# mokemokechicken/reversi-alpha-zero

Hardware: AMD Instinct MI355X
Metric: MCTS simulations/sec (self-play, NN included) (higher is better)
Workload: dtype f64 tree statistics + f32 net (f16x3 split-operand MFMA trunk)

## Files before the change

### reversi-alpha-zero_amd/csrc/raz_net_f16x3.hip

```cpp
#include <hip/hip_runtime.h>
#include <math.h>
#include <stdlib.h>
#include <string.h>
#include <vector>
#include "raz_bitboard.h"
#include "raz_detmath.h"
#include "raz_internal.h"
#include "raz_net_heads.h"
#include "raz_net_layout.h"

namespace {

typedef _Float16 h8 __attribute__((ext_vector_type(8)));
typedef _Float16 h4 __attribute__((ext_vector_type(4)));
typedef float f32x4 __attribute__((ext_vector_type(4)));
typedef float f32x16 __attribute__((ext_vector_type(16)));

constexpr int OCT = 128;
constexpr int NWAVE = 8;
constexpr int W_STAGE = 3 * 2 * 2 * OCT * 16;
constexpr int ACT_POS = 4 * 64 * 16;
constexpr int Z_OFF = NWAVE * (ACT_POS + 128);
constexpr int Z_BYTES = 2048;
constexpr int ACT_IMG = Z_OFF + Z_BYTES;
constexpr int LDS_W = 0;
constexpr int LDS_ACT = 2 * W_STAGE;
constexpr int LDS_BYTES = LDS_ACT + 2 * ACT_IMG;
constexpr int act_pos_off(int p) { return p * (ACT_POS + 128); }

#ifdef RAZ_F16X3_STAMPS
#define RAZ_STAMP_PARAM , unsigned long long* __restrict__ stamps
#define RAZ_STAMP_ARG , (unsigned long long*)nullptr
#define RAZ_STAMP_BEGIN                                                                                           \
    unsigned long long st_t[8];                                                                                   \
    st_t[0] = __builtin_amdgcn_s_memtime();                                                                       \
    st_t[7] = __builtin_amdgcn_s_memrealtime();                                                                   \
    st_t[6] = (unsigned long long)__builtin_amdgcn_s_getreg((4 << 0) | (0 << 6) | (31 << 11)) | ((unsigned long long)__builtin_amdgcn_s_getreg((20 << 0) | (0 << 6) | (31 << 11)) << 32); \
    st_t[5] = 0;                                                                                                  \
    st_t[1] = st_t[2] = st_t[3] = st_t[4] = 0;                                                                    \
    unsigned long long st_b = 0
#define RAZ_STAMP_BARRIER_IN st_b = __builtin_amdgcn_s_memtime()
#define RAZ_STAMP_BARRIER_OUT(st_)                                    \
    do {                                                              \
        const unsigned long long t_ = __builtin_amdgcn_s_memtime();   \
        st_t[5] += t_ - st_b;                                         \
        if ((st_) == 0) st_t[1] = t_;                                 \
    } while (0)
#define RAZ_STAMP_AT(i_) st_t[i_] = __builtin_amdgcn_s_memtime()
#define RAZ_STAMP_END                                                                                    \
    do {                                                                                                 \
        st_t[3] = __builtin_amdgcn_s_memtime();                                                          \
        __builtin_amdgcn_s_waitcnt(0x0070);                                                \
        st_t[4] = __builtin_amdgcn_s_memtime();                                                          \
        if (lane == 0 && stamps)                                                                         \
            for (int i_ = 0; i_ < 8; ++i_) stamps[((size_t)blockIdx.x * NWAVE + wv) * 8 + i_] = st_t[i_]; \
    } while (0)
#else
#define RAZ_STAMP_PARAM
#define RAZ_STAMP_ARG
#define RAZ_STAMP_BEGIN
#define RAZ_STAMP_BARRIER_IN
#define RAZ_STAMP_BARRIER_OUT(st_)
#define RAZ_STAMP_AT(i_)
#define RAZ_STAMP_END
#endif

__device__ __forceinline__ void halves_trade(float a, float b, int upper, float& first, float& second) {
#ifdef RAZ_WAVE_EMU
    const float got = __shfl_xor(upper ? a : b, 32);
    first = upper ? got : a;
    second = upper ? b : got;
#else
    (void)upper;
    const auto r = __builtin_amdgcn_permlane32_swap(__float_as_uint(a), __float_as_uint(b), false, false);
    first = __uint_as_float(r[0]);
    second = __uint_as_float(r[1]);
#endif
}

#define GLDS16(gptr, lptr)                                                                                      \
    __builtin_amdgcn_global_load_lds((const __attribute__((address_space(1))) void*)(gptr),                     \
                                     (__attribute__((address_space(3))) void*)(lptr), 16, 0, 0)

template <bool SPLIT, int TG, int J0, int J1>
__device__ __forceinline__ void conv_stage(const unsigned char* lds, uint32_t wbase, uint32_t abase, const uint32_t (&boff)[3],
                                           f32x16 (&acc)[2][4]) {
#pragma unroll
    for (int tt = 0; tt < 3; ++tt) {
        h8 bh[4], bl[4];
#pragma unroll
        for (int j = J0; j < J1; ++j) {
            const uint32_t at = abase + boff[tt] + (j + TG) * 128;
            bh[j] = *(const h8*)(lds + at);
            if constexpr (SPLIT) bl[j] = *(const h8*)(lds + at + 1024);
        }
#pragma unroll
        for (int m = 0; m < 2; ++m) {
            const h8 ah = *(const h8*)(lds + wbase + tt * 8192 + m * 512);
            if constexpr (SPLIT) {
                const h8 al = *(const h8*)(lds + wbase + tt * 8192 + m * 512 + 2048);
#pragma unroll
                for (int j = J0; j < J1; ++j) {
                    acc[m][j] = __builtin_amdgcn_mfma_f32_32x32x16_f16(al, bh[j], acc[m][j], 0, 0, 0);
                    acc[m][j] = __builtin_amdgcn_mfma_f32_32x32x16_f16(ah, bl[j], acc[m][j], 0, 0, 0);
                    acc[m][j] = __builtin_amdgcn_mfma_f32_32x32x16_f16(ah, bh[j], acc[m][j], 0, 0, 0);
                }
            } else {
#pragma unroll
                for (int j = J0; j < J1; ++j) acc[m][j] = __builtin_amdgcn_mfma_f32_32x32x16_f16(ah, bh[j], acc[m][j], 0, 0, 0);
            }
        }
    }
}

template <bool SPLIT>
__global__ __launch_bounds__(512, 2) void k_conv3x3_f16x3(const unsigned char* __restrict__ Wl, const float* __restrict__ bias,
                                                          const float* __restrict__ inv_scale_ptr, const unsigned char* in, unsigned char* out,
                                                          const unsigned char* skip, const uint8_t* __restrict__ active, int n, int F,
                                                          unsigned* __restrict__ flag, const uint32_t* __restrict__ n_ptr RAZ_STAMP_PARAM) {
    extern __shared__ __attribute__((aligned(16))) unsigned char lds[];
    const int tid = threadIdx.x, lane = tid & 63;
    const int wv = __builtin_amdgcn_readfirstlane(tid >> 6);
    RAZ_STAMP_BEGIN;
    if (n_ptr) n = (int)*n_ptr < n ? (int)*n_ptr : n;
    const int noct = F / OCT, nchunks = F / 16;
    const int b = blockIdx.x;
    const int ot = (b >> 3) % noct;
    const int pg = (b / (8 * noct)) * 8 + (b & 7);
    const int p0 = pg * NWAVE, pos = p0 + wv;
    if (p0 >= n) return;
    const size_t pos_bytes = (size_t)F * 256;
    const unsigned char* in_pos = in + (size_t)(pos < n ? pos : n - 1) * pos_bytes;
    if (tid < 2 * (Z_BYTES / 16)) {
        const int im = tid / (Z_BYTES / 16), k = tid % (Z_BYTES / 16);
        ((f32x4*)(lds + LDS_ACT + im * ACT_IMG + Z_OFF))[k] = (f32x4){0.f, 0.f, 0.f, 0.f};
    }
    const int half = wv >> 2, grp = (wv >> 1) & 1, oh = wv & 1;
    const int kg = lane >> 5, colpos = grp * 4 + ((lane & 31) >> 3), x = lane & 7;
    uint32_t boff[3];
#pragma unroll
    for (int t = 0; t < 3; ++t) {
        const int xx = x + t - 1;
        const int at = act_pos_off(colpos) + kg * 2048 + ((4 * half - 1) * 8 + xx) * 16;
        boff[t] = xx >= 0 && xx < 8 ? (uint32_t)at : (uint32_t)(Z_OFF + (at & 255));
    }
    const uint32_t aoff = (uint32_t)(kg * 4096 + oh * 1024 + (lane & 31) * 16);
    f32x16 acc[2][4];
#pragma unroll
    for (int m = 0; m < 2; ++m)
#pragma unroll
        for (int j = 0; j < 4; ++j)
#pragma unroll
            for (int r = 0; r < 16; ++r) acc[m][j][r] = 0.f;
    const unsigned char* wsrc = Wl + (size_t)ot * nchunks * 3 * W_STAGE + lane * 16;
    const unsigned char* asrc = in_pos + lane * 16;
    auto issue = [&](int c, int tg) {
        const int st = c * 3 + tg;
        const unsigned char* src = wsrc + (size_t)st * W_STAGE;
        unsigned char* dst = lds + LDS_W + (st & 1) * W_STAGE;
        if constexpr (SPLIT) {
#pragma unroll
            for (int i = 0; i < 3; ++i) GLDS16(src + (wv * 3 + i) * 1024, dst + (wv * 3 + i) * 1024);
        } else {
            const int p0w = (wv >> 1) * 4 + (wv & 1);
            GLDS16(src + p0w * 1024, dst + p0w * 1024);
            if (wv < 4) GLDS16(src + (p0w + 16) * 1024, dst + (p0w + 16) * 1024);
        }
        if (tg == 0) {
            const unsigned char* a = asrc + (size_t)c * ACT_POS;
            unsigned char* ad = lds + LDS_ACT + (c & 1) * ACT_IMG + act_pos_off(wv);
#pragma unroll
            for (int pl = 0; pl < 4; pl += SPLIT ? 1 : 2) GLDS16(a + pl * 1024, ad + pl * 1024);
        }
    };
    issue(0, 0);
    for (int c = 0; c < nchunks; ++c) {
        const uint32_t abase = (uint32_t)(LDS_ACT + (c & 1) * ACT_IMG);
#pragma unroll
        for (int tg = 0; tg < 3; ++tg) {
            const int st = c * 3 + tg;
            RAZ_STAMP_BARRIER_IN;
            __syncthreads();
            RAZ_STAMP_BARRIER_OUT(st);
            if (tg < 2) issue(c, tg + 1);
            else if (c + 1 < nchunks) issue(c + 1, 0);
            const uint32_t wbase = (uint32_t)(LDS_W + (st & 1) * W_STAGE) + aoff;
            if (tg == 0) {
                conv_stage<SPLIT, 0, 1, 4>(lds, wbase, abase, boff, acc);
                if (half != 0) conv_stage<SPLIT, 0, 0, 1>(lds, wbase, abase, boff, acc);
            } else if (tg == 1) {
                conv_stage<SPLIT, 1, 0, 4>(lds, wbase, abase, boff, acc);
            } else {
                conv_stage<SPLIT, 2, 0, 3>(lds, wbase, abase, boff, acc);
                if (half != 1) conv_stage<SPLIT, 2, 3, 4>(lds, wbase, abase, boff, acc);
            }
        }
    }
    RAZ_STAMP_AT(2);
    const int lpos = p0 + colpos;
    const bool live = lpos < n && (!active || active[lpos]);
    if (!__any(live)) return;
    const float inv_scale = *inv_scale_ptr;
    const size_t lane_off = (size_t)(live ? lpos : p0) * pos_bytes + (size_t)((4 * half + kg) * 8 + x) * 16;
    unsigned char* out_pos = out + lane_off;
    const unsigned char* skip_pos = skip ? skip + lane_off : nullptr;
    h8 skh[2][4], skl[2][4];
    auto load_skip = [&](int it) {
#pragma unroll
        for (int q = 0; q < 4; ++q) {
            const int oc8 = ot * OCT + oh * 64 + (it >> 1) * 32 + q * 8;
            const size_t unit = (size_t)(oc8 >> 4) * ACT_POS + (size_t)((oc8 >> 3) & 1) * 2048 + (size_t)(it & 1) * 256;
            skh[it & 1][q] = *(const h8*)(skip_pos + unit);
            if constexpr (SPLIT) skl[it & 1][q] = *(const h8*)(skip_pos + unit + 1024);
        }
    };
    if (skip_pos && live) load_skip(0);
    bool over = false;
#pragma unroll
    for (int it = 0; it < 4; ++it) {
        const int m = it >> 1, k = it & 1;
        if (skip_pos && live && it + 1 < 4) load_skip(it + 1);
#pragma unroll
        for (int q = 0; q < 4; ++q) {
            const int oc8 = ot * OCT + oh * 64 + m * 32 + q * 8;
            const size_t unit = (size_t)(oc8 >> 4) * ACT_POS + (size_t)((oc8 >> 3) & 1) * 2048 + (size_t)k * 256;
            float v[8];
#pragma unroll
            for (int j = 0; j < 4; ++j) halves_trade(acc[m][2 * k][q * 4 + j], acc[m][2 * k + 1][q * 4 + j], kg, v[j], v[4 + j]);
            if (!live) continue;
#pragma unroll
            for (int j = 0; j < 8; ++j) v[j] = v[j] * inv_scale + bias[oc8 + j];
            if (skip_pos) {
                const h8 sh = skh[it & 1][q];
                if constexpr (SPLIT) {
                    const h8 sl = skl[it & 1][q];
#pragma unroll
                    for (int j = 0; j < 8; ++j) v[j] = v[j] + ((float)sh[j] + (float)sl[j]);
                } else {
#pragma unroll
                    for (int j = 0; j < 8; ++j) v[j] = v[j] + (float)sh[j];
                }
            }
            h8 hi, lo;
#pragma unroll
            for (int j = 0; j < 8; ++j) {
                const float r = v[j] > 0.0f ? v[j] : 0.0f;
                over |= !(r < 60000.0f);
                hi[j] = (_Float16)r;
                lo[j] = (_Float16)(r - (float)hi[j]);
            }
            *(h8*)(out_pos + unit) = hi;
            if constexpr (SPLIT) *(h8*)(out_pos + unit + 1024) = lo;
        }
    }
    if (live && over) flag[(size_t)lpos * RAZ_NET_ROWFLAG_WORDS] = 1u;
    RAZ_STAMP_END;
}

typedef float f32x2 __attribute__((ext_vector_type(2)));
constexpr int CONV0_ROWS = 2;

template <bool SPLIT>
__global__ __launch_bounds__(256, 6) void k_conv0_split(const float* __restrict__ W0, const raz_bb* __restrict__ own,
                                                        const raz_bb* __restrict__ enemy, const uint8_t* __restrict__ active,
                                                        unsigned char* out, int n, int F, unsigned* __restrict__ flag,
                                                        const uint32_t* __restrict__ list, const uint32_t* __restrict__ n_ptr) {
    const int posA = blockIdx.x * CONV0_ROWS, posB = posA + 1, lane = threadIdx.x & 63;
    const int wv = __builtin_amdgcn_readfirstlane(threadIdx.x >> 6);
    if (threadIdx.x == 0) {
        flag[(size_t)posA * RAZ_NET_ROWFLAG_WORDS] = 0u;
        if (posB < n) flag[(size_t)posB * RAZ_NET_ROWFLAG_WORDS] = 0u;
        if (posA == 0) flag[1] = 0u;
    }
    __syncthreads();
    if (n_ptr) n = (int)*n_ptr < n ? (int)*n_ptr : n;
    const bool liveA = posA < n && (list || !active || active[posA]);
    const bool liveB = posB < n && (list || !active || active[posB]);
    if (!liveA && !liveB) return;
    raz_bb bo[2] = {0, 0}, be[2] = {0, 0};
    if (liveA) {
        const size_t src = list ? list[posA] : (size_t)posA;
        bo[0] = own[src];
        be[0] = enemy[src];
    }
    if (liveB) {
        const size_t src = list ? list[posB] : (size_t)posB;
        bo[1] = own[src];
        be[1] = enemy[src];
    }
    f32x2 x0[9], x1[9];
#pragma unroll
    for (int t = 0; t < 9; ++t) {
        int s;
        const bool ok = bb_tap(lane, t, &s);
#pragma unroll
        for (int k = 0; k < 2; ++k) {
            x0[t][k] = ok ? (float)(uint32_t)((bo[k] >> s) & 1) : 0.0f;
            x1[t][k] = ok ? (float)(uint32_t)((be[k] >> s) & 1) : 0.0f;
        }
    }
    const float* bias = W0 + (size_t)F * 18;
    unsigned char* op = out + (size_t)posA * F * 256 + lane * 16;
    bool overA = false, overB = false;
    for (int ocb = wv; ocb < F / 16; ocb += 4) {
#pragma unroll 1
        for (int g = 0; g < 2; ++g) {
            f32x2 acc[8];
#pragma unroll
            for (int o = 0; o < 8; ++o) {
                const float b = bias[ocb * 16 + g * 8 + o];
                acc[o] = (f32x2){b, b};
            }
#pragma unroll
            for (int t = 0; t < 9; ++t) {
                const float* wt = W0 + ((size_t)ocb * 9 + t) * 32 + g * 8;
#pragma unroll
                for (int o = 0; o < 8; ++o) {
                    const float w = wt[o];
                    acc[o] = __builtin_elementwise_fma(x0[t], (f32x2){w, w}, acc[o]);
                }
#pragma unroll
                for (int o = 0; o < 8; ++o) {
                    const float w = wt[16 + o];
                    acc[o] = __builtin_elementwise_fma(x1[t], (f32x2){w, w}, acc[o]);
                }
            }
#pragma unroll
            for (int k = 0; k < 2; ++k) {
                if (!(k ? liveB : liveA)) continue;
                h8 hi, lo;
                bool over = false;
#pragma unroll
                for (int j = 0; j < 8; ++j) {
                    const float r = acc[j][k] > 0.0f ? acc[j][k] : 0.0f;
                    over |= !(r < 60000.0f);
                    hi[j] = (_Float16)r;
                    lo[j] = (_Float16)(r - (float)hi[j]);
                }
                if (k) overB |= over;
                else overA |= over;
                unsigned char* o16 = op + (size_t)k * F * 256 + (size_t)ocb * ACT_POS + (g * 2) * 1024;
                *(h8*)o16 = hi;
                if constexpr (SPLIT) *(h8*)(o16 + 1024) = lo;
            }
        }
    }
    if (overA) flag[(size_t)posA * RAZ_NET_ROWFLAG_WORDS] = 1u;
    if (overB) flag[(size_t)posB * RAZ_NET_ROWFLAG_WORDS] = 1u;
}

template <bool SPLIT>
__global__ __launch_bounds__(64) void k_heads_split(const float* __restrict__ H, const unsigned char* trunk,
                                                    const uint8_t* __restrict__ active, float* __restrict__ policy,
                                                    float* __restrict__ value, int n, int F, int V,
                                                    const uint32_t* __restrict__ list, const uint32_t* __restrict__ n_ptr) {
    extern __shared__ __attribute__((aligned(16))) float head[];
    const int pos = blockIdx.x, lane = threadIdx.x;
    if (n_ptr) n = (int)*n_ptr < n ? (int)*n_ptr : n;
    if (pos >= n || (!list && active && !active[pos])) return;
    const size_t dst = list ? list[pos] : (size_t)pos;
    const HeadWeights h = head_weights(H, F, V);
    const unsigned char* a = trunk + (size_t)pos * F * 256 + lane * 16;
    float p0 = h.pol_b[0], p1 = h.pol_b[1], v0 = h.val_b[0];
    for (int c = 0; c < F / 16; ++c) {
#pragma unroll
        for (int g = 0; g < 2; ++g) {
            const h8 hi = *(const h8*)(a + (size_t)c * ACT_POS + (g * 2 + 0) * 1024);
            h8 lo = hi;
            if constexpr (SPLIT) lo = *(const h8*)(a + (size_t)c * ACT_POS + (g * 2 + 1) * 1024);
#pragma unroll
            for (int j = 0; j < 8; ++j)
                heads_1x1_step(h, F, c * 16 + g * 8 + j, SPLIT ? (float)hi[j] + (float)lo[j] : (float)hi[j], p0, p1, v0);
        }
    }
    heads_finish(h, V, p0, p1, v0, head, lane, policy + dst * 64, value + dst);
}

}

void raz_net_build_f16x3(const float* src, float* dst, int F, int R, int V) {
    const float* lsrc = src + ((size_t)F * 18 + F);
    float* scales = dst + f16x3_scale_off(F, R, V);
    const int nchunks = F / 16, noct = F / 128;
    for (int l = 1; l < 2 * R + 1; ++l) {
        float mx = 0.f;
        for (size_t i = 0; i < (size_t)F * F * 9; ++i) mx = fmaxf(mx, fabsf(lsrc[i]));
        int e = 0;
        if (mx > 0.f) frexpf(mx, &e);
        const float S = ldexpf(1.0f, 15 - e);
        scales[l - 1] = ldexpf(1.0f, e - 15);
        _Float16* w = (_Float16*)(dst + f16x3_layer_off(F, R, V, l));
        for (int ot = 0; ot < noct; ++ot)
            for (int c = 0; c < nchunks; ++c)
                for (int t = 0; t < 9; ++t)
                    for (int kg = 0; kg < 2; ++kg)
                        for (int o = 0; o < 128; ++o)
                            for (int j = 0; j < 8; ++j) {
                                const int oc = ot * 128 + o, ic = c * 16 + kg * 8 + j;
                                const float v = lsrc[((size_t)oc * F + ic) * 9 + t] * S;
                                const _Float16 hi = (_Float16)v, lo = (_Float16)(v - (float)hi);
                                const size_t stage = ((size_t)ot * nchunks + c) * 3 + t / 3;
                                const size_t base = stage * (W_STAGE / 2) + ((size_t)(t % 3) * 2 + kg) * 2 * 128 * 8;
                                w[base + (size_t)o * 8 + j] = hi;
                                w[base + 128 * 8 + (size_t)o * 8 + j] = lo;
                            }
        lsrc += (size_t)F * F * 9 + F;
    }
}

static int heads_launch(bool split, const float* W, int F, int R, int V, const unsigned char* trunk, const uint8_t* active, float* policy,
                        float* value, size_t n, hipStream_t s, const uint32_t* list, const uint32_t* n_ptr) {
    const auto heads = split ? k_heads_split<true> : k_heads_split<false>;
    hipLaunchKernelGGL(heads, dim3((unsigned)n), dim3(64), heads_lds_floats(V) * sizeof(float), s,
                       W + heads_off(F, R), trunk, active, policy, value, (int)n, F, V, list, n_ptr);
    return raz_check_launch("raz_net_forward (split heads)");
}
int raz_net_heads_split(const float* W, int F, int R, int V, const unsigned char* trunk, const uint8_t* active, float* policy, float* value,
                        size_t n, hipStream_t s, const uint32_t* list, const uint32_t* n_ptr) {
    return heads_launch(true, W, F, R, V, trunk, active, policy, value, n, s, list, n_ptr);
}

size_t raz_net_f16x3_scratch_bytes(int F, size_t n) { return n * ((size_t)2 * F * 256 + RAZ_NET_ROWFLAG_WORDS * 4); }

__global__ __launch_bounds__(256) void k_flag_unrepaired(const unsigned* __restrict__ rowflag, unsigned* __restrict__ sticky, int n,
                                                         const uint32_t* __restrict__ n_ptr) {
    const int i = blockIdx.x * 256 + threadIdx.x;
    const int rows = n_ptr ? ((int)*n_ptr < n ? (int)*n_ptr : n) : n;
    if (i < rows && rowflag[(size_t)i * RAZ_NET_ROWFLAG_WORDS]) atomicOr(sticky, 1u);
}
static int raz_net_flag_unrepaired(const unsigned* rowflag, unsigned* sticky, size_t n, const uint32_t* n_ptr, hipStream_t s) {
    hipLaunchKernelGGL(k_flag_unrepaired, dim3((unsigned)((n + 255) / 256)), dim3(256), 0, s, rowflag, sticky, (int)n, n_ptr);
    return raz_check_launch("raz_net_forward (range flags)");
}

unsigned* raz_net_f16x3_flag(const float* W, int F, int R, int V) { return (unsigned*)(W + f16x3_scale_off(F, R, V) + (size_t)2 * R + 8); }

int raz_net_forward_f16x3(const float* W, int F, int R, int V, const uint64_t* own, const uint64_t* enemy,
                          const uint8_t* active, float* policy, float* value, size_t n, void* scratch, size_t scratch_bytes,
                          hipStream_t s, const uint32_t* list, const uint32_t* n_ptr, bool split) {
    if (!scratch || scratch_bytes < raz_net_f16x3_scratch_bytes(F, n))
        return raz_fail(RAZ_ENOMEM, "raz_net_forward: scratch too small (raz_net_scratch_bytes)");
    unsigned char* bufA = (unsigned char*)scratch;
    unsigned char* bufT = bufA + (size_t)n * F * 256;
    unsigned* sticky = raz_net_f16x3_flag(W, F, R, V);
    unsigned* flag = (unsigned*)(bufT + (size_t)n * F * 256);
    const float* scales = W + f16x3_scale_off(F, R, V);
    const auto conv = split ? k_conv3x3_f16x3<true> : k_conv3x3_f16x3<false>;
    if (const int rc = raz_lds_opt_in((const void*)conv, LDS_BYTES, "raz_net_forward: hipFuncSetAttribute")) return rc;
    const unsigned conv_threads = NWAVE * 64;
    const auto conv0 = split ? k_conv0_split<true> : k_conv0_split<false>;
    hipLaunchKernelGGL(conv0, dim3((unsigned)((n + CONV0_ROWS - 1) / CONV0_ROWS)), dim3(256), 0, s, W + conv_off(F, 0), (const raz_bb*)own,
                       (const raz_bb*)enemy, active, bufA, (int)n, F, flag, list, n_ptr);
    const unsigned groups = (unsigned)((n + NWAVE - 1) / NWAVE);
    const unsigned tiles = ((groups + 7) / 8) * 8 * (unsigned)(F / 128);
    const unsigned grid = tiles;
    for (int r = 0; r < R; ++r) {
        const int l1 = 1 + 2 * r, l2 = 2 + 2 * r;
        hipLaunchKernelGGL(conv, dim3(grid), dim3(conv_threads), LDS_BYTES, s,
                           (const unsigned char*)(W + f16x3_layer_off(F, R, V, l1)), W + conv_off(F, l1) + (size_t)F * 9 * F,
                           scales + (l1 - 1), (const unsigned char*)bufA, bufT, (const unsigned char*)nullptr, list ? nullptr : active, (int)n, F, flag, n_ptr RAZ_STAMP_ARG);
        hipLaunchKernelGGL(conv, dim3(grid), dim3(conv_threads), LDS_BYTES, s,
                           (const unsigned char*)(W + f16x3_layer_off(F, R, V, l2)), W + conv_off(F, l2) + (size_t)F * 9 * F,
                           scales + (l2 - 1), (const unsigned char*)bufT, bufA, (const unsigned char*)bufA, list ? nullptr : active, (int)n, F, flag, n_ptr RAZ_STAMP_ARG);
    }
    const int rc = heads_launch(split, W, F, R, V, bufA, active, policy, value, n, s, list, n_ptr);
    if (rc != RAZ_OK) return rc;
    if (!f16x3_repairs(F, V))
        return raz_net_flag_unrepaired(flag, sticky, n, n_ptr, s);
    return raz_net_repair_rows(W, F, R, V, own, enemy, policy, value, n, flag, sticky, list, n_ptr, s);
}
```

Baseline: 389,900.

## Triple-buffer conv weights and software-pipeline LDS reads with MFMAs

Adds a third weight stage buffer so each tap group has a dedicated LDS slot, and restructures the chunk loop so the weights for the next stage are prefetched further ahead. Inside each stage, LDS operand reads for the next tap are interleaved with the MFMAs of the current tap, with scheduling barriers, so that LDS latency is hidden behind matrix math. The cost is more LDS use, which may reduce occupancy, higher register pressure from holding several operand sets at once, and a more complex barrier schedule.

After: 400,500, median of 6. +2.7%, better.

```diff
diff --git a/reversi-alpha-zero_amd/csrc/raz_net_f16x3.hip b/reversi-alpha-zero_amd/csrc/raz_net_f16x3.hip
--- a/reversi-alpha-zero_amd/csrc/raz_net_f16x3.hip
+++ b/reversi-alpha-zero_amd/csrc/raz_net_f16x3.hip
@@ -24,7 +24,7 @@
 constexpr int Z_BYTES = 2048;
 constexpr int ACT_IMG = Z_OFF + Z_BYTES;
 constexpr int LDS_W = 0;
-constexpr int LDS_ACT = 2 * W_STAGE;
+constexpr int LDS_ACT = 3 * W_STAGE;
 constexpr int LDS_BYTES = LDS_ACT + 2 * ACT_IMG;
 constexpr int act_pos_off(int p) { return p * (ACT_POS + 128); }
 
@@ -82,6 +82,69 @@
     __builtin_amdgcn_global_load_lds((const __attribute__((address_space(1))) void*)(gptr),                     \
                                      (__attribute__((address_space(3))) void*)(lptr), 16, 0, 0)
 
+struct TapOps {
+    h8 bh[4], bl[4], ah[2], al[2];
+};
+
+template <bool SPLIT, int TG, int J0, int J1>
+__device__ __forceinline__ void tap_read(const unsigned char* lds, uint32_t wtap, uint32_t btap, int k, TapOps& p) {
+    constexpr int R = J1 - J0;
+    if constexpr (SPLIT) {
+        if (k == 0) p.al[0] = *(const h8*)(lds + wtap + 2048);
+        else if (k == 2) p.ah[0] = *(const h8*)(lds + wtap);
+        else if (k == 2 * R + 2) p.al[1] = *(const h8*)(lds + wtap + 512 + 2048);
+        else if (k == 2 * R + 3) p.ah[1] = *(const h8*)(lds + wtap + 512);
+        else {
+            const int b = k == 1 ? 0 : k == 3 ? 1 : k - 2;
+            const int j = J0 + (b >> 1);
+            if (b & 1) p.bl[j] = *(const h8*)(lds + btap + (j + TG) * 128 + 1024);
+            else p.bh[j] = *(const h8*)(lds + btap + (j + TG) * 128);
+        }
+    } else {
+        if (k == 0) p.ah[0] = *(const h8*)(lds + wtap);
+        else if (k == R + 1) p.ah[1] = *(const h8*)(lds + wtap + 512);
+        else p.bh[J0 + k - 1] = *(const h8*)(lds + btap + (J0 + k - 1 + TG) * 128);
+    }
+}
+template <bool SPLIT, int R>
+constexpr int tap_reads() { return SPLIT ? 2 * R + 4 : R + 2; }
+
+template <bool SPLIT, int J0, int J1>
+__device__ __forceinline__ void tap_mfma(const TapOps& p, int q, f32x16 (&acc)[2][4]) {
+    constexpr int R = J1 - J0;
+    if constexpr (SPLIT) {
+        const int m = q / (3 * R), j = J0 + (q / 3) % R, term = q % 3;
+        acc[m][j] = __builtin_amdgcn_mfma_f32_32x32x16_f16(term == 0 ? p.al[m] : p.ah[m], term == 1 ? p.bl[j] : p.bh[j], acc[m][j], 0, 0, 0);
+    } else {
+        const int m = q / R, j = J0 + q % R;
+        acc[m][j] = __builtin_amdgcn_mfma_f32_32x32x16_f16(p.ah[m], p.bh[j], acc[m][j], 0, 0, 0);
+    }
+}
+template <bool SPLIT, int R>
+constexpr int tap_mfmas() { return SPLIT ? 6 * R : 2 * R; }
+
+template <bool SPLIT, int J0, int J1, int NTG, int NJ0, int NJ1>
+__device__ __forceinline__ void tap_pipelined(const unsigned char* lds, const TapOps& cur, TapOps& nxt, uint32_t nwtap, uint32_t nbtap,
+                                              f32x16 (&acc)[2][4]) {
+    constexpr int NL = tap_reads<SPLIT, NJ1 - NJ0>(), NM = tap_mfmas<SPLIT, J1 - J0>();
+#pragma unroll
+    for (int i = 0; i < NL; ++i) {
+        tap_read<SPLIT, NTG, NJ0, NJ1>(lds, nwtap, nbtap, i, nxt);
+#pragma unroll
+        for (int q = i * (NM - NM / 4) / NL; q < (i + 1 < NL ? (i + 1) * (NM - NM / 4) / NL : NM); ++q) tap_mfma<SPLIT, J0, J1>(cur, q, acc);
+        __builtin_amdgcn_sched_barrier(0);
+    }
+}
+
+template <bool SPLIT, int TG, int J0, int J1, int NTG, int NJ0, int NJ1>
+__device__ __forceinline__ void conv_stage_main(const unsigned char* lds, uint32_t wbase, uint32_t abase, uint32_t nwbase, uint32_t nabase,
+                                                const uint32_t (&boff)[3], f32x16 (&acc)[2][4], TapOps& ops) {
+    TapOps t1, t2;
+    tap_pipelined<SPLIT, J0, J1, TG, J0, J1>(lds, ops, t1, wbase + 8192, abase + boff[1], acc);
+    tap_pipelined<SPLIT, J0, J1, TG, J0, J1>(lds, t1, t2, wbase + 2 * 8192, abase + boff[2], acc);
+    tap_pipelined<SPLIT, J0, J1, NTG, NJ0, NJ1>(lds, t2, ops, nwbase, nabase + boff[0], acc);
+}
+
 template <bool SPLIT, int TG, int J0, int J1>
 __device__ __forceinline__ void conv_stage(const unsigned char* lds, uint32_t wbase, uint32_t abase, const uint32_t (&boff)[3],
                                            f32x16 (&acc)[2][4]) {
@@ -154,10 +217,9 @@
             for (int r = 0; r < 16; ++r) acc[m][j][r] = 0.f;
     const unsigned char* wsrc = Wl + (size_t)ot * nchunks * 3 * W_STAGE + lane * 16;
     const unsigned char* asrc = in_pos + lane * 16;
-    auto issue = [&](int c, int tg) {
-        const int st = c * 3 + tg;
-        const unsigned char* src = wsrc + (size_t)st * W_STAGE;
-        unsigned char* dst = lds + LDS_W + (st & 1) * W_STAGE;
+    auto issue_w = [&](int c, int tg) {
+        const unsigned char* src = wsrc + (size_t)(c * 3 + tg) * W_STAGE;
+        unsigned char* dst = lds + LDS_W + tg * W_STAGE;
         if constexpr (SPLIT) {
 #pragma unroll
             for (int i = 0; i < 3; ++i) GLDS16(src + (wv * 3 + i) * 1024, dst + (wv * 3 + i) * 1024);
@@ -166,34 +228,47 @@
             GLDS16(src + p0w * 1024, dst + p0w * 1024);
             if (wv < 4) GLDS16(src + (p0w + 16) * 1024, dst + (p0w + 16) * 1024);
         }
-        if (tg == 0) {
-            const unsigned char* a = asrc + (size_t)c * ACT_POS;
-            unsigned char* ad = lds + LDS_ACT + (c & 1) * ACT_IMG + act_pos_off(wv);
-#pragma unroll
-            for (int pl = 0; pl < 4; pl += SPLIT ? 1 : 2) GLDS16(a + pl * 1024, ad + pl * 1024);
-        }
     };
-    issue(0, 0);
+    auto issue_a = [&](int c) {
+        const unsigned char* a = asrc + (size_t)c * ACT_POS;
+        unsigned char* ad = lds + LDS_ACT + (c & 1) * ACT_IMG + act_pos_off(wv);
+#pragma unroll
+        for (int pl = 0; pl < 4; pl += SPLIT ? 1 : 2) GLDS16(a + pl * 1024, ad + pl * 1024);
+    };
+    const uint32_t w0 = (uint32_t)LDS_W + aoff, w1 = w0 + W_STAGE, w2 = w1 + W_STAGE;
+    issue_w(0, 0);
+    issue_a(0);
+    issue_w(0, 1);
+    RAZ_STAMP_BARRIER_IN;
+    __syncthreads();
+    RAZ_STAMP_BARRIER_OUT(0);
+    TapOps ops;
+#pragma unroll
+    for (int k = 0; k < tap_reads<SPLIT, 3>(); ++k) tap_read<SPLIT, 0, 1, 4>(lds, w0, (uint32_t)LDS_ACT + boff[0], k, ops);
     for (int c = 0; c < nchunks; ++c) {
-        const uint32_t abase = (uint32_t)(LDS_ACT + (c & 1) * ACT_IMG);
-#pragma unroll
-        for (int tg = 0; tg < 3; ++tg) {
-            const int st = c * 3 + tg;
+        const uint32_t abase = (uint32_t)(LDS_ACT + (c & 1) * ACT_IMG), nabase = (uint32_t)(LDS_ACT + (~c & 1) * ACT_IMG);
+        const bool more = c + 1 < nchunks;
+        issue_w(c, 2);
+        conv_stage_main<SPLIT, 0, 1, 4, 1, 0, 4>(lds, w0, abase, w1, abase, boff, acc, ops);
+        if (half != 0) conv_stage<SPLIT, 0, 0, 1>(lds, w0, abase, boff, acc);
+        RAZ_STAMP_BARRIER_IN;
+        __syncthreads();
+        RAZ_STAMP_BARRIER_OUT(3 * c + 1);
+        if (more) {
+            issue_w(c + 1, 0);
+            issue_a(c + 1);
+        }
+        conv_stage_main<SPLIT, 1, 0, 4, 2, 0, 3>(lds, w1, abase, w2, abase, boff, acc, ops);
+        RAZ_STAMP_BARRIER_IN;
+        __syncthreads();
+        RAZ_STAMP_BARRIER_OUT(3 * c + 2);
+        if (more) issue_w(c + 1, 1);
+        conv_stage_main<SPLIT, 2, 0, 3, 0, 1, 4>(lds, w2, abase, w0, nabase, boff, acc, ops);
+        if (half != 1) conv_stage<SPLIT, 2, 3, 4>(lds, w2, abase, boff, acc);
+        if (more) {
             RAZ_STAMP_BARRIER_IN;
             __syncthreads();
-            RAZ_STAMP_BARRIER_OUT(st);
-            if (tg < 2) issue(c, tg + 1);
-            else if (c + 1 < nchunks) issue(c + 1, 0);
-            const uint32_t wbase = (uint32_t)(LDS_W + (st & 1) * W_STAGE) + aoff;
-            if (tg == 0) {
-                conv_stage<SPLIT, 0, 1, 4>(lds, wbase, abase, boff, acc);
-                if (half != 0) conv_stage<SPLIT, 0, 0, 1>(lds, wbase, abase, boff, acc);
-            } else if (tg == 1) {
-                conv_stage<SPLIT, 1, 0, 4>(lds, wbase, abase, boff, acc);
-            } else {
-                conv_stage<SPLIT, 2, 0, 3>(lds, wbase, abase, boff, acc);
-                if (half != 1) conv_stage<SPLIT, 2, 3, 4>(lds, wbase, abase, boff, acc);
-            }
+            RAZ_STAMP_BARRIER_OUT(3 * c + 3);
         }
     }
     RAZ_STAMP_AT(2);
```
